# TUMFTM/global_racetrajectory_optimization

Hardware: AMD Instinct MI355X
Metric: min-curv QP solves/sec, N=2000 waypoints, batch=1024 per GPU (higher is better)
Workload: dtype f64

## Files before the change

global_racetrajectory_optimization_amd/csrc/mcq_kernels.hip:

```cpp
#include "mcq_kernels.h"

#include <math.h>



#define MCQ_NT 256
#define MCQ_NW (MCQ_NT / 64)
typedef double d2 __attribute__((vector_size(16)));
typedef __attribute__((address_space(1))) d2 gd2;

#define SM_RED 0
#define SM_S (SM_RED + 64)
#define SPK 1920
#define SM_OVL (SM_S + SPK)
#define OVL_SIZE 7464
#define SM_KV (SM_OVL + OVL_SIZE)
#define SM_KI (SM_KV + 3 * MCQ_KMAX)
#define SM_TOTAL (SM_KI + (3 * MCQ_KMAX + 2 + 1) / 2 + 1)
static_assert(sizeof(double) * SM_TOTAL <= 80 * 1024, "two workgroups of the solver kernel per CU");

size_t mcq_solve_lds_bytes() { return sizeof(double) * SM_TOTAL; }

__shared__ double g_sm[SM_TOTAL];

// ... 425 lines not shown
    if (c.direct) { (void)sp_solve(c, v, v); return; }
    if (c.kkt_f32) solve_kkt<true>(c, v, fwd_done);
    else solve_kkt<false>(c, v, fwd_done);
}

__device__ __forceinline__ void apply_Et(const LCtx& c, const gdouble* src, gdouble* dst) { tri_apply_Et(c, src, dst); }

__device__ __noinline__ void gradient(const LCtx& c, const gdouble* x, const gdouble* extra, gdouble* tmp, gdouble* g)
{
    const int n = c.d.n;
    const long long t0 = TICK();
    __syncthreads();
    if (c.direct) {
        const gdouble* HD = VEC(c.w, c.nm, V_SPD);
        const gdouble* HU = VEC(c.w, c.nm, V_SPU);
        const gdouble* F = VEC(c.w, c.nm, V_F);
        for (int i = threadIdx.x; i < n; i += MCQ_NT) {
            const int im = i > 0 ? i - 1 : n - 1, ip = i + 1 < n ? i + 1 : 0;
            g[i] = F[i] + HU[im] * x[im] + HD[i] * x[i] + HU[i] * x[ip];
        }
        __syncthreads();
        if (threadIdx.x == 0) c.tk[2] += TICK() - t0;
        return;
    }
    tri_apply_E(c, x, VEC(c.w, c.nm, V_KREF), MCQ_F_SCALE, tmp);
    if (extra) {
        for (int i = threadIdx.x; i < n; i += MCQ_NT) tmp[i] += extra[i];
        __syncthreads();
    }
    tri_apply_Et(c, tmp, g);
    if (threadIdx.x == 0) c.tk[2] += TICK() - t0;
}

__device__ __forceinline__ int timed_factor(const LCtx& c, const gdouble* sig, const gschar* mk, gdouble* fv = nullptr, bool f32 = false)
{
    const long long t0 = TICK();
    const int r = factor(c, sig, mk, fv, f32);
    if (threadIdx.x == 0) c.tk[0] += TICK() - t0;
    return r;
}
__device__ __forceinline__ void timed_solve(const LCtx& c, gdouble* v, bool fwd_done = false)
{
    const long long t0 = TICK();
    solve(c, v, fwd_done);
    if (threadIdx.x == 0) c.tk[1] += TICK() - t0;
}


__device__ __noinline__ int ipm(const LCtx& c, bool with_kappa)
{
    const int tid = threadIdx.x, n = c.d.n, nm = c.nm;
    double* red = g_sm + SM_RED;
    const gdouble* LO = VEC(c.w, nm, V_LO);
    const gdouble* HI = VEC(c.w, nm, V_HI);
    const gdouble* KR = VEC(c.w, nm, V_KREF);
    gdouble* X = VEC(c.w, nm, V_X);
    gdouble* G = VEC(c.w, nm, V_G);
    gdouble* ZL = VEC(c.w, nm, V_ZL);
    gdouble* ZU = VEC(c.w, nm, V_ZU);
    gdouble* SIG = VEC(c.w, nm, V_SIG);
    gdouble* RHS = VEC(c.w, nm, V_RHS);
    gdouble* DXA = VEC(c.w, nm, V_DXA);
    gdouble* T0 = VEC(c.w, nm, V_T0);
    gdouble* T1 = VEC(c.w, nm, V_T1);
    gdouble* T2 = VEC(c.w, nm, V_T2);
    gdouble* TL = VEC(c.w, nm, V_TL);
    gdouble* TU = VEC(c.w, nm, V_TU);
    gdouble* YL = VEC(c.w, nm, V_YL);
    gdouble* YU = VEC(c.w, nm, V_YU);
    gdouble* SK = VEC(c.w, nm, V_SK);
    gdouble* EDA = VEC(c.w, nm, V_EDA);
    gdouble* Q = VEC(c.w, nm, V_Q);
    gschar* ST = c.w.state;
    const double kb = c.kbound, zscale = c.zscale;
    const double IPM_TOL = 1e-10;
    c.out_iters = 0;

    for (int i = tid; i < n; i += MCQ_NT) {
        const bool fixed = !(HI[i] - LO[i] > 1e-12);
        ST[i] = fixed ? 2 : 0;
        X[i] = 0.5 * (LO[i] + HI[i]);
        ZL[i] = fixed ? 0.0 : zscale;
        ZU[i] = ZL[i];
    }
    __syncthreads();
    if (with_kappa) {
        tri_apply_E(c, X, KR, 1.0, T0);
        const double mu0 = 0.5 * zscale * c.wmean;
        for (int i = tid; i < n; i += MCQ_NT) {
            const double r = T0[i];
            const double tl = fmax(kb + r, 0.1 * kb), tu = fmax(kb - r, 0.1 * kb);
            TL[i] = tl; TU[i] = tu;
            YL[i] = mu0 / tl; YU[i] = mu0 / tu;
        }
        __syncthreads();
    }
    const double npairs = 2.0 * c.nfree + (with_kappa ? 2.0 * n : 0.0);
    const gschar* const no_mask = nullptr;
    const bool any_fixed = c.nfree < (double)n;
    (void)no_mask;
    if (!(npairs > 0.0)) return MCQ_OK;

    bool g_exact = true;
    double mu_first = 0.0, rdm_best = 1e300;
    for (int it = 1; it <= c.max_ipm_iter; ++it) {
        if (with_kappa) {
            for (int i = tid; i < n; i += MCQ_NT) Q[i] = YU[i] - YL[i];
            gradient(c, X, Q, T0, T1);
            gradient(c, X, nullptr, T0, G);
            tri_apply_E(c, X, KR, 1.0, T0);
        }
        double mu, rdm, rhom;
        for (;;) {
            mu = 0.0; rdm = 0.0; rhom = 0.0;
            for (int i = tid; i < n; i += MCQ_NT) {
                if (with_kappa) {
                    mu += TL[i] * YL[i] + TU[i] * YU[i];
                    rhom = fmax(rhom, fmax(fabs(TL[i] - (kb + T0[i])), fabs(TU[i] - (kb - T0[i]))));
                    SK[i] = YL[i] / TL[i] + YU[i] / TU[i];
                }
                if (ST[i] != 0) continue;
                const double sl = X[i] - LO[i], su = HI[i] - X[i];
                mu += sl * ZL[i] + su * ZU[i];
                const double gg = with_kappa ? T1[i] : G[i];
                rdm = fmax(rdm, fabs(gg - ZL[i] + ZU[i]));
                SIG[i] = ZL[i] / sl + ZU[i] / su;
            }
            mu = block_reduce_(mu, 0, red) / npairs;
            rdm = block_reduce_(rdm, 2, red);
            rhom = block_reduce_(rhom, 2, red);
            const bool conv = mu < IPM_TOL * zscale * c.wmean && rdm < IPM_TOL * zscale && rhom <= 1e-9 * kb;
            if (with_kappa && it > 1 && mu < 1e-6 * mu_first && rdm > 10.0 * rdm_best) return MCQ_OK;
            rdm_best = fmin(rdm_best, rdm);
#ifdef IPM_TRACE
            if (tid == 0) printf("ipm%d it %d mu %.3e rdm %.3e rhom %.3e step %.3e\n", (int)with_kappa, it, mu / (zscale * c.wmean), rdm / zscale, rhom / kb, c.last_step);
#endif
            if (conv && (with_kappa || g_exact)) return MCQ_OK;
            if (!conv) break;
            gradient(c, X, nullptr, T0, G);
            g_exact = true;
        }
        c.out_iters = it;
        if (it == 1) mu_first = mu;

        int fs;
        if (with_kappa) {
            for (int i = tid; i < n; i += MCQ_NT) EDA[i] = 1.0 + SK[i];
            __syncthreads();
            c.kkt_w = EDA;
            fs = timed_factor(c, SIG, any_fixed ? ST : nullptr);
            c.kkt_w = nullptr;
            if (fs == MCQ_NOT_PD && mu < 1e-6 * mu_first) return MCQ_OK;
        } else {
            fs = timed_factor(c, SIG, any_fixed ? ST : nullptr);
        }
        if (fs != 0) return fs;

        if (with_kappa) {
            for (int i = tid; i < n; i += MCQ_NT) {
                const double rl = TL[i] - (kb + T0[i]), ru = TU[i] - (kb - T0[i]);
                Q[i] = YL[i] * rl / TL[i] - YU[i] * ru / TU[i];
            }
            __syncthreads();
            apply_Et(c, Q, T2);
            __syncthreads();
            for (int i = tid; i < n; i += MCQ_NT) RHS[i] = ST[i] == 0 ? -G[i] + T2[i] : 0.0;
        } else {
            for (int i = tid; i < n; i += MCQ_NT) RHS[i] = ST[i] == 0 ? -G[i] : 0.0;
        }
        timed_solve(c, RHS);
        if (with_kappa) {
            tri_apply_E(c, RHS, nullptr, 0.0, EDA);
        }
        double ap = 1.0, ad = 1.0;
        for (int i = tid; i < n; i += MCQ_NT) {
            if (with_kappa) {
                const double rl = TL[i] - (kb + T0[i]), ru = TU[i] - (kb - T0[i]);
                const double dtl = EDA[i] - rl, dtu = -EDA[i] - ru;
                const double dyl = -YL[i] - YL[i] * dtl / TL[i], dyu = -YU[i] - YU[i] * dtu / TU[i];
                if (dtl < 0.0) ap = fmin(ap, -TL[i] / dtl);
                if (dtu < 0.0) ap = fmin(ap, -TU[i] / dtu);
                if (dyl < 0.0) ad = fmin(ad, -YL[i] / dyl);
                if (dyu < 0.0) ad = fmin(ad, -YU[i] / dyu);
            }
            if (ST[i] != 0) { DXA[i] = 0.0; continue; }
            const double dx = RHS[i];
            DXA[i] = dx;
            const double sl = X[i] - LO[i], su = HI[i] - X[i];
            const double dzl = -ZL[i] - ZL[i] * dx / sl, dzu = -ZU[i] + ZU[i] * dx / su;
            if (dx < 0.0) ap = fmin(ap, -sl / dx);
            if (dx > 0.0) ap = fmin(ap, su / dx);
            if (dzl < 0.0) ad = fmin(ad, -ZL[i] / dzl);
            if (dzu < 0.0) ad = fmin(ad, -ZU[i] / dzu);
        }
        ap = block_reduce_(ap, 1, red);
        ad = block_reduce_(ad, 1, red);
        double mua = 0.0;
        for (int i = tid; i < n; i += MCQ_NT) {
            if (with_kappa) {
                const double rl = TL[i] - (kb + T0[i]), ru = TU[i] - (kb - T0[i]);
                const double dtl = EDA[i] - rl, dtu = -EDA[i] - ru;
                const double dyl = -YL[i] - YL[i] * dtl / TL[i], dyu = -YU[i] - YU[i] * dtu / TU[i];
                mua += (TL[i] + ap * dtl) * (YL[i] + ad * dyl) + (TU[i] + ap * dtu) * (YU[i] + ad * dyu);
            }
            if (ST[i] != 0) continue;
            const double dx = DXA[i];
            const double sl = X[i] - LO[i], su = HI[i] - X[i];
            const double dzl = -ZL[i] - ZL[i] * dx / sl, dzu = -ZU[i] + ZU[i] * dx / su;
            mua += (sl + ap * dx) * (ZL[i] + ad * dzl) + (su - ap * dx) * (ZU[i] + ad * dzu);
        }
        mua = block_reduce_(mua, 0, red) / npairs;
        const double ratio = mua / mu;
        const double smu = ratio * ratio * ratio * mu;

        if (with_kappa) {
            for (int i = tid; i < n; i += MCQ_NT) {
                const double rl = TL[i] - (kb + T0[i]), ru = TU[i] - (kb - T0[i]);
                const double dtl = EDA[i] - rl, dtu = -EDA[i] - ru;
                const double dyl = -YL[i] - YL[i] * dtl / TL[i], dyu = -YU[i] - YU[i] * dtu / TU[i];
                Q[i] = (smu - dtl * dyl + YL[i] * rl) / TL[i] - (smu - dtu * dyu + YU[i] * ru) / TU[i];
            }
            __syncthreads();
            apply_Et(c, Q, T2);
            __syncthreads();
        }
        for (int i = tid; i < n; i += MCQ_NT) {
            if (ST[i] != 0) { RHS[i] = 0.0; continue; }
            const double dx = DXA[i];
            const double sl = X[i] - LO[i], su = HI[i] - X[i];
            const double dzl = -ZL[i] - ZL[i] * dx / sl, dzu = -ZU[i] + ZU[i] * dx / su;
            RHS[i] = -G[i] + (smu - dx * dzl) / sl - (smu + dx * dzu) / su + (with_kappa ? T2[i] : 0.0);
        }
        timed_solve(c, RHS);
        if (with_kappa) {
            tri_apply_E(c, RHS, nullptr, 0.0, Q);
        }
        double amax = 1.0 / 0.995;
        for (int i = tid; i < n; i += MCQ_NT) {
            if (with_kappa) {
                const double rl = TL[i] - (kb + T0[i]), ru = TU[i] - (kb - T0[i]);
                const double dtla = EDA[i] - rl, dtua = -EDA[i] - ru;
                const double dyla = -YL[i] - YL[i] * dtla / TL[i], dyua = -YU[i] - YU[i] * dtua / TU[i];
                const double dtl = Q[i] - rl, dtu = -Q[i] - ru;
                const double dyl = (-TL[i] * YL[i] + smu - dtla * dyla - YL[i] * dtl) / TL[i];
                const double dyu = (-TU[i] * YU[i] + smu - dtua * dyua - YU[i] * dtu) / TU[i];
                EDA[i] = dyl;
                SK[i] = dyu;
                if (dtl < 0.0) amax = fmin(amax, -TL[i] / dtl);
                if (dtu < 0.0) amax = fmin(amax, -TU[i] / dtu);
                if (dyl < 0.0) amax = fmin(amax, -YL[i] / dyl);
                if (dyu < 0.0) amax = fmin(amax, -YU[i] / dyu);
            }
            if (ST[i] != 0) continue;
            const double dx = RHS[i], da = DXA[i];
            const double sl = X[i] - LO[i], su = HI[i] - X[i];
            const double dzla = -ZL[i] - ZL[i] * da / sl, dzua = -ZU[i] + ZU[i] * da / su;
            const double dzl = (-sl * ZL[i] + smu - da * dzla - ZL[i] * dx) / sl;
            const double dzu = (-su * ZU[i] + smu + da * dzua + ZU[i] * dx) / su;
            T1[i] = dzl;
            T2[i] = dzu;
            if (dx < 0.0) amax = fmin(amax, -sl / dx);
            if (dx > 0.0) amax = fmin(amax, su / dx);
            if (dzl < 0.0) amax = fmin(amax, -ZL[i] / dzl);
            if (dzu < 0.0) amax = fmin(amax, -ZU[i] / dzu);
        }
        amax = block_reduce_(amax, 1, red);
        const double a = fmin(1.0, 0.995 * amax);
        c.last_step = a;
        for (int i = tid; i < n; i += MCQ_NT) {
            if (with_kappa) {
                const double rl = TL[i] - (kb + T0[i]), ru = TU[i] - (kb - T0[i]);
                TL[i] += a * (Q[i] - rl);
                TU[i] += a * (-Q[i] - ru);
                YL[i] += a * EDA[i];
                YU[i] += a * SK[i];
            }
            if (ST[i] != 0) continue;
            if (!with_kappa) {
                const double dxa = DXA[i], dx = RHS[i];
                const double sl = X[i] - LO[i], su = HI[i] - X[i];
                const double dzla = -ZL[i] - ZL[i] * dxa / sl, dzua = -ZU[i] + ZU[i] * dxa / su;
                const double rc = -G[i] + (smu - dxa * dzla) / sl - (smu + dxa * dzua) / su;
                G[i] += a * (rc - SIG[i] * dx);
            }
            {
                const double sl = X[i] - LO[i], su = HI[i] - X[i];
                const double rsl = (sl + a * RHS[i]) * ZL[i], rzl = (ZL[i] + a * T1[i]) * sl;
                const double rsu = (su - a * RHS[i]) * ZU[i], rzu = (ZU[i] + a * T2[i]) * su;
                const bool al = rsl < MCQ_TAPIA_RATIO * rzl && sl + a * RHS[i] < MCQ_TAPIA_SHRINK * sl, au = rsu < MCQ_TAPIA_RATIO * rzu && su - a * RHS[i] < MCQ_TAPIA_SHRINK * su;
                VEC(c.w, nm, V_T3)[i] = al ? -1.0 : (au ? 1.0 : 0.0);
            }
            X[i] += a * RHS[i];
            ZL[i] += a * T1[i];
            ZU[i] += a * T2[i];
        }
        g_exact = false;
        __syncthreads();
    }
    return with_kappa ? MCQ_KAPPA_INFEASIBLE : MCQ_ITER_CAP;
}

#define IPB_E 8
#define IPB_H 4
__device__ __noinline__ int ipm_box(const LCtx& c, double tol, bool resume)
{
#define IPB_SETUP                                                                                                      \
    const int tid = threadIdx.x, n = c.d.n, nm = c.nm;                                                                 \
    double* red = g_sm + SM_RED;                                                                                       \
    const gdouble* LO = VEC(c.w, nm, V_LO);                                                                            \
    const gdouble* HI = VEC(c.w, nm, V_HI);                                                                            \
    gdouble* X = VEC(c.w, nm, V_X);                                                                                    \
    gdouble* G = VEC(c.w, nm, V_G);                                                                                    \
    gdouble* ZL = VEC(c.w, nm, V_ZL);                                                                                  \
    gdouble* ZU = VEC(c.w, nm, V_ZU);                                                                                  \
    gdouble* SIG = VEC(c.w, nm, V_SIG);                                                                                \
    gdouble* RHS = VEC(c.w, nm, V_RHS);                                                                                \
    gdouble* DXA = VEC(c.w, nm, V_DXA);                                                                                \
    gschar* ST = c.w.state;                                                                                            \
    gdouble* IND = VEC(c.w, nm, V_T3);                                                                                 \
    (void)IND; (void)red; (void)LO; (void)HI; (void)X; (void)G; (void)ZL; (void)ZU; (void)SIG; (void)RHS; (void)DXA; (void)ST;    \
    int idx[IPB_E];                                                                                                    \
    bool ok[IPB_E];                                                                                                    \
    _Pragma("unroll") for (int u = 0; u < IPB_E; ++u) {                                                                \
        ok[u] = tid + u * MCQ_NT < n;                                                                                  \
        idx[u] = ok[u] ? tid + u * MCQ_NT : 0;           \
    }
#define IPB_HALF(h)                                                                                                    \
    int idx[IPB_H];                                                                                                    \
    bool ok[IPB_H];                                                                                                    \
    _Pragma("unroll") for (int u = 0; u < IPB_H; ++u) {                                                                \
        ok[u] = tid + ((h) * IPB_H + u) * MCQ_NT < n;                                                                  \
        idx[u] = ok[u] ? tid + ((h) * IPB_H + u) * MCQ_NT : 0;                                                         \
    }
#define IPB_PTRS                                                                                                       \
    const int tid = threadIdx.x, n = c.d.n, nm = c.nm;                                                                 \
    double* red = g_sm + SM_RED;                                                                                       \
    const gdouble* LO = VEC(c.w, nm, V_LO);                                                                            \
    const gdouble* HI = VEC(c.w, nm, V_HI);                                                                            \
    gdouble* X = VEC(c.w, nm, V_X);                                                                                    \
    gdouble* G = VEC(c.w, nm, V_G);                                                                                    \
    gdouble* ZL = VEC(c.w, nm, V_ZL);                                                                                  \
    gdouble* ZU = VEC(c.w, nm, V_ZU);                                                                                  \
    gdouble* SIG = VEC(c.w, nm, V_SIG);                                                                                \
    gdouble* RHS = VEC(c.w, nm, V_RHS);                                                                                \
    gdouble* DXA = VEC(c.w, nm, V_DXA);                                                                                \
    gschar* ST = c.w.state;                                                                                            \
    gdouble* IND = VEC(c.w, nm, V_T3);                                                                                 \
    (void)IND; (void)red; (void)LO; (void)HI; (void)X; (void)G; (void)ZL; (void)ZU; (void)SIG; (void)RHS; (void)DXA; (void)ST;
    const double zscale = c.zscale;
    const double IPM_TOL = tol;
    c.out_iters = 0;
    {
    IPB_SETUP
#pragma unroll
    for (int u = 0; u < IPB_E; ++u) {
        if (!ok[u]) continue;
        const int i = idx[u];
        const bool fixed = !(HI[i] - LO[i] > 1e-12);
        ST[i] = fixed ? 2 : 0;
        if (!resume) {
            X[i] = 0.5 * (LO[i] + HI[i]);
            ZL[i] = fixed ? 0.0 : zscale;
            ZU[i] = ZL[i];
        }
    }
    }
    __syncthreads();
    if (resume) gradient(c, VEC(c.w, c.nm, V_X), nullptr, VEC(c.w, c.nm, V_T0), VEC(c.w, c.nm, V_G));
    const double npairs = 2.0 * c.nfree;
    const bool any_fixed = c.nfree < (double)c.d.n;
    if (!(npairs > 0.0)) return MCQ_OK;

    bool g_exact = true;
    double mu_prev = 1e300;
    int stalled = 0;
#ifndef MCQ_IPM_F32
#define MCQ_IPM_F32 1
#endif
#ifndef MCQ_IPM_F32_RD
#define MCQ_IPM_F32_RD 1e-5
#endif
    bool f32 = MCQ_IPM_F32 && !resume;
#ifndef MCQ_IPM_TRUST_FP64_CARRY
#define MCQ_IPM_TRUST_FP64_CARRY 1
#endif
    bool g_f32 = false;
    for (int it = 1; it <= c.max_ipm_iter; ++it) {
        double mu;
        for (;;) {
            IPB_PTRS
            double rdm = 0.0;
            mu = 0.0;
            {
#pragma unroll
            for (int h = 0; h < IPB_E / IPB_H; ++h) {
                IPB_HALF(h)
                double x[IPB_H], lo[IPB_H], hi[IPB_H], zl[IPB_H], zu[IPB_H], g[IPB_H];
                int st[IPB_H];
#pragma unroll
                for (int u = 0; u < IPB_H; ++u) {
                    const int i = idx[u];
                    st[u] = ST[i]; x[u] = X[i]; lo[u] = LO[i]; hi[u] = HI[i]; zl[u] = ZL[i]; zu[u] = ZU[i]; g[u] = G[i];
                }
#pragma unroll
                for (int u = 0; u < IPB_H; ++u) {
                    if (!ok[u]) continue;
                    const int i = idx[u];
                    if (st[u] != 0) { RHS[i] = 0.0; continue; }
                    const double sl = x[u] - lo[u], su = hi[u] - x[u];
                    mu += sl * zl[u] + su * zu[u];
                    rdm = fmax(rdm, fabs(g[u] - zl[u] + zu[u]));
                    SIG[i] = zl[u] / sl + zu[u] / su;
                    RHS[i] = -g[u];
                }
            }
            block_reduce2_(mu, 0, rdm, 2, red);
            mu /= npairs;
            }
            const bool conv = mu < IPM_TOL * zscale * c.wmean && rdm < IPM_TOL * zscale;
#ifdef IPM_TRACE
            if (threadIdx.x == 0) printf("ipmb it %d mu %.3e rdm %.3e exact %d resume %d\n", it, mu / (zscale * c.wmean), rdm / zscale, (int)g_exact, (int)resume);
#endif
            if (f32 && it > 1 && rdm < MCQ_IPM_F32_RD * zscale) {
                f32 = false;
                if (!g_exact) {
                    gradient(c, X, nullptr, VEC(c.w, nm, V_T0), G);
                    g_exact = true;
                    g_f32 = false;
                    continue;
                }
            }
            if (conv && (g_exact || (MCQ_IPM_TRUST_FP64_CARRY && !resume && !g_f32))) return MCQ_OK;
            if (!conv) break;
            gradient(c, X, nullptr, VEC(c.w, nm, V_T0), G);
            g_exact = true;
            g_f32 = false;
        }
        c.out_iters = it;
        if (resume) {
            stalled = mu > 0.9 * mu_prev ? stalled + 1 : 0;
            mu_prev = mu;
            if (stalled >= 3) return MCQ_OK;
        }

        const int fs = timed_factor(c, VEC(c.w, c.nm, V_SIG), any_fixed ? c.w.state : nullptr,
                                    VEC(c.w, c.nm, V_RHS), f32);
        if (fs != 0) return (resume && fs == MCQ_NOT_PD) ? MCQ_OK : fs;
        timed_solve(c, VEC(c.w, c.nm, V_RHS), true);

        double smu;
        {
            IPB_SETUP
            double dxa[IPB_E], sl[IPB_E], su[IPB_E], zl[IPB_E], zu[IPB_E], g[IPB_E];
            bool act[IPB_E];
#pragma unroll
            for (int u = 0; u < IPB_E; ++u) {
                const int i = idx[u];
                const double x = X[i];
                act[u] = ok[u] && ST[i] == 0;
                dxa[u] = RHS[i]; sl[u] = x - LO[i]; su[u] = HI[i] - x; zl[u] = ZL[i]; zu[u] = ZU[i]; g[u] = G[i];
            }
            double ap = 1.0, ad = 1.0;
#pragma unroll
            for (int u = 0; u < IPB_E; ++u) {
                if (!ok[u]) continue;
                if (!act[u]) { DXA[idx[u]] = 0.0; continue; }
                const double dx = dxa[u];
                DXA[idx[u]] = dx;
                const double dzla = -zl[u] - zl[u] * dx / sl[u];
                const double dzua = -zu[u] + zu[u] * dx / su[u];
                if (dx < 0.0) ap = fmin(ap, -sl[u] / dx);
                if (dx > 0.0) ap = fmin(ap, su[u] / dx);
                if (dzla < 0.0) ad = fmin(ad, -zl[u] / dzla);
                if (dzua < 0.0) ad = fmin(ad, -zu[u] / dzua);
            }
            block_reduce2_(ap, 1, ad, 1, red);
            double mua = 0.0;
#pragma unroll
            for (int u = 0; u < IPB_E; ++u) {
                if (!act[u]) continue;
                const double dzla = -zl[u] - zl[u] * dxa[u] / sl[u];
                const double dzua = -zu[u] + zu[u] * dxa[u] / su[u];
                mua += (sl[u] + ap * dxa[u]) * (zl[u] + ad * dzla) + (su[u] - ap * dxa[u]) * (zu[u] + ad * dzua);
            }
            mua = block_reduce_(mua, 0, red) / npairs;
            const double ratio = mua / mu;
            smu = ratio * ratio * ratio * mu;
#pragma unroll
            for (int u = 0; u < IPB_E; ++u) {
                if (!ok[u]) continue;
                const double dzla = -zl[u] - zl[u] * dxa[u] / sl[u];
                const double dzua = -zu[u] + zu[u] * dxa[u] / su[u];
                RHS[idx[u]] = act[u] ? -g[u] + (smu - dxa[u] * dzla) / sl[u] - (smu + dxa[u] * dzua) / su[u] : 0.0;
            }
        }
        timed_solve(c, VEC(c.w, c.nm, V_RHS));

        {
            IPB_SETUP
#ifdef MCQ_IPM_FIXED_STEP
            const double gm = 0.995;
#else
            const double gm = fmin(fmax(MCQ_IPM_GM_MIN, 1.0 - MCQ_IPM_GM_C * mu / (zscale * c.wmean)), 1.0 - 1e-9);
#endif
            double amax = 1.0 / gm;
            double dx[IPB_E], da[IPB_E], x[IPB_E], lo[IPB_E], hi[IPB_E], zl[IPB_E], zu[IPB_E], g[IPB_E], sg[IPB_E];
            bool act[IPB_E];
#pragma unroll
            for (int u = 0; u < IPB_E; ++u) {
                const int i = idx[u];
                act[u] = ok[u] && ST[i] == 0;
                dx[u] = RHS[i]; da[u] = DXA[i]; x[u] = X[i]; lo[u] = LO[i]; hi[u] = HI[i]; zl[u] = ZL[i]; zu[u] = ZU[i];
                g[u] = G[i]; sg[u] = SIG[i];
            }
#define IPB_STEP3(u)                                                                                                          \
                const double sl = x[u] - lo[u], su = hi[u] - x[u];                                                              \
                const double dzla = -zl[u] - zl[u] * da[u] / sl, dzua = -zu[u] + zu[u] * da[u] / su;                             \
                const double dzl = (-sl * zl[u] + smu - da[u] * dzla - zl[u] * dx[u]) / sl;                                     \
                const double dzu = (-su * zu[u] + smu + da[u] * dzua + zu[u] * dx[u]) / su;
#pragma unroll
            for (int u = 0; u < IPB_E; ++u) {
                if (!act[u]) continue;
                IPB_STEP3(u)
                if (dx[u] < 0.0) amax = fmin(amax, -sl / dx[u]);
                if (dx[u] > 0.0) amax = fmin(amax, su / dx[u]);
                if (dzl < 0.0) amax = fmin(amax, -zl[u] / dzl);
                if (dzu < 0.0) amax = fmin(amax, -zu[u] / dzu);
            }
            amax = block_reduce_(amax, 1, red);
            const double a = fmin(1.0, gm * amax);
            c.last_step = a;
#pragma unroll
            for (int u = 0; u < IPB_E; ++u) {
                if (!act[u]) continue;
                const int i = idx[u];
                IPB_STEP3(u)
                const double rc = -g[u] + (smu - da[u] * dzla) / sl - (smu + da[u] * dzua) / su;
                const double hdx = rc - sg[u] * dx[u];
                const double gn = g[u] + a * hdx, xn = x[u] + a * dx[u], zln = zl[u] + a * dzl, zun = zu[u] + a * dzu;
                G[i] = gn;
                X[i] = xn;
                ZL[i] = zln;
                ZU[i] = zun;
                const double rsl = (sl + a * dx[u]) * zl[u], rzl = (zl[u] + a * dzl) * sl;
                const double rsu = (su - a * dx[u]) * zu[u], rzu = (zu[u] + a * dzu) * su;
                const bool al = rsl < MCQ_TAPIA_RATIO * rzl && sl + a * dx[u] < MCQ_TAPIA_SHRINK * sl, au = rsu < MCQ_TAPIA_RATIO * rzu && su - a * dx[u] < MCQ_TAPIA_SHRINK * su;
                IND[i] = al ? -1.0 : (au ? 1.0 : 0.0);
            }
#undef IPB_STEP3
        }
        g_exact = false;
        g_f32 |= f32;
        __syncthreads();
    }
    return MCQ_ITER_CAP;
#undef IPB_SETUP
}

struct KappaMem {
    double* kmu;
    double* krh;
    double* mul;
    int* ki;
    int* piv;
    gdouble* sg;
    int cap, ld;
    bool in_lds;
};
__device__ __forceinline__ KappaMem kappa_mem_lds(const LCtx& c)
{
    KappaMem k;
    k.kmu = g_sm + SM_KV;
    k.krh = g_sm + SM_KV + MCQ_KMAX;
    k.mul = g_sm + SM_KV + 2 * MCQ_KMAX;
    k.ki = (int*)(g_sm + SM_KI);
    k.piv = (int*)(g_sm + SM_KI) + 1 + 2 * MCQ_KMAX;
    k.sg = c.w.Z + c.nm;
    k.cap = MCQ_KMAX;
    k.ld = MCQ_KMAX;
    k.in_lds = true;
    return k;
}
__device__ __forceinline__ KappaMem kappa_mem_slot(double* slot)
{
    KappaMem k;
    k.sg = (gdouble*)slot;
    double* v = slot + (size_t)MCQ_KBIG * MCQ_KBIG;
    k.kmu = v;
    k.krh = v + MCQ_KBIG;
    k.mul = v + 2 * MCQ_KBIG;
    k.ki = (int*)(v + 3 * MCQ_KBIG);
    k.piv = k.ki + 2 + 2 * MCQ_KBIG;
    k.cap = MCQ_KBIG;
    k.ld = MCQ_KBIG;
    k.in_lds = false;
    return k;
}

template <typename PA>
__device__ __forceinline__ void kappa_lu_eliminate(PA A, int lda, int nk, double* mul, int* piv)
{
    const int tid = threadIdx.x;
    double* red = g_sm + SM_RED;
    for (int cidx = 0; cidx < nk; ++cidx) {
        double best = -1.0;
        int brow = cidx;
        for (int r = cidx + tid; r < nk; r += MCQ_NT) {
            const double v = fabs(A[(size_t)r * lda + cidx]);
            if (v > best) { best = v; brow = r; }
        }
        const double bmax = block_reduce_(best, 2, red);
        double cand = (best == bmax && best >= 0.0) ? (double)brow : 1e300;
        cand = block_reduce_(cand, 1, red);
        const int pr = cand < 1e299 ? (int)cand : cidx;
        if (tid == 0) piv[cidx] = pr;
        if (pr != cidx)
            for (int cc = tid; cc < nk; cc += MCQ_NT) {
                const double t = A[(size_t)cidx * lda + cc];
                A[(size_t)cidx * lda + cc] = A[(size_t)pr * lda + cc];
                A[(size_t)pr * lda + cc] = t;
            }
        __syncthreads();
        const double pv = A[(size_t)cidx * lda + cidx];
        for (int r = cidx + 1 + tid; r < nk; r += MCQ_NT) mul[r] = pv != 0.0 ? A[(size_t)r * lda + cidx] / pv : 0.0;
        __syncthreads();
        const int rem = nk - cidx - 1;
        for (int e = tid; e < rem * rem; e += MCQ_NT) {
            const int r = cidx + 1 + e / rem, cc = cidx + 1 + e % rem;
            A[(size_t)r * lda + cc] -= mul[r] * A[(size_t)cidx * lda + cc];
        }
        __syncthreads();
        for (int r = cidx + 1 + tid; r < nk; r += MCQ_NT) A[(size_t)r * lda + cidx] = mul[r];
        __syncthreads();
    }
}

__device__ void kappa_lu_factor(const KappaMem& K, int nk)
{
    const int tid = threadIdx.x;
    __syncthreads();
    if (K.in_lds && nk * nk <= OVL_SIZE) {
        double* A = g_sm + SM_OVL;
        for (int e = tid; e < nk * nk; e += MCQ_NT) A[e] = K.sg[(size_t)(e / nk) * K.ld + (e % nk)];
        __syncthreads();
        kappa_lu_eliminate(A, nk, nk, K.mul, K.piv);
        for (int e = tid; e < nk * nk; e += MCQ_NT) K.sg[(size_t)(e / nk) * K.ld + (e % nk)] = A[e];
    } else {
        kappa_lu_eliminate(K.sg, K.ld, nk, K.mul, K.piv);
    }
    __syncthreads();
}

template <typename PA>
__device__ __forceinline__ void kappa_lu_substitute(PA A, int lda, int nk, double* KMU, const int* piv)
{
    const int tid = threadIdx.x;
    if (tid == 0)
        for (int cidx = 0; cidx < nk; ++cidx) {
            const int pr = piv[cidx];
            if (pr != cidx) { const double t = KMU[cidx]; KMU[cidx] = KMU[pr]; KMU[pr] = t; }
        }
    __syncthreads();
    for (int cidx = 0; cidx < nk; ++cidx) {
        const double yc = KMU[cidx];
        __syncthreads();
        for (int r = cidx + 1 + tid; r < nk; r += MCQ_NT) KMU[r] -= A[(size_t)r * lda + cidx] * yc;
        __syncthreads();
    }
    for (int cidx = nk - 1; cidx >= 0; --cidx) {
        if (tid == 0) { const double pv = A[(size_t)cidx * lda + cidx]; KMU[cidx] = pv != 0.0 ? KMU[cidx] / pv : 0.0; }
        __syncthreads();
        const double xc = KMU[cidx];
        for (int r = tid; r < cidx; r += MCQ_NT) KMU[r] -= A[(size_t)r * lda + cidx] * xc;
        __syncthreads();
    }
}

__device__ void kappa_lu_solve(const KappaMem& K, int nk)
{
    const int tid = threadIdx.x;
    __syncthreads();
    for (int q = tid; q < nk; q += MCQ_NT) K.kmu[q] = K.krh[q];
    if (K.in_lds && nk * nk <= OVL_SIZE) {
        double* A = g_sm + SM_OVL;
        for (int e = tid; e < nk * nk; e += MCQ_NT) A[e] = K.sg[(size_t)(e / nk) * K.ld + (e % nk)];
        __syncthreads();
        kappa_lu_substitute((const double*)A, nk, nk, K.kmu, K.piv);
    } else {
        __syncthreads();
        kappa_lu_substitute((const gdouble*)K.sg, K.ld, nk, K.kmu, K.piv);
    }
}

__device__ void kappa_apply(const LCtx& c, const KappaMem& K, int nk, gdouble* Q, gdouble* v)
{
    const int tid = threadIdx.x, n = c.d.n;
    const double* KMU = K.kmu;
    const int* KI = K.ki;
    const gschar* ST = c.w.state;
    for (int i = tid; i < n; i += MCQ_NT) Q[i] = 0.0;
    __syncthreads();
    for (int q = tid; q < nk; q += MCQ_NT) Q[KI[1 + q]] = KMU[q];
    __syncthreads();
    apply_Et(c, Q, v);
    __syncthreads();
    for (int i = tid; i < n; i += MCQ_NT) if (ST[i] != 0) v[i] = 0.0;
    __syncthreads();
    timed_solve(c, v);
}

__device__ __noinline__ int active_set(const LCtx& c, bool with_kappa, bool tapia, int cap, int identify, const KappaMem K)
{
    const int tid = threadIdx.x, n = c.d.n, nm = c.nm;
    double* red = g_sm + SM_RED;
    double* KMU = K.kmu;
    double* KRH = K.krh;
    int* KI = K.ki;
    const int kcap = K.cap;
    const gdouble* LO = VEC(c.w, nm, V_LO);
    const gdouble* HI = VEC(c.w, nm, V_HI);
    const gdouble* KR = VEC(c.w, nm, V_KREF);
    gdouble* X = VEC(c.w, nm, V_X);
    gdouble* G = VEC(c.w, nm, V_G);
    gdouble* ZL = VEC(c.w, nm, V_ZL);
    gdouble* ZU = VEC(c.w, nm, V_ZU);
    gdouble* RHS = VEC(c.w, nm, V_RHS);
    gdouble* T0 = VEC(c.w, nm, V_T0);
    gdouble* T1 = VEC(c.w, nm, V_T1);
    gdouble* T2 = VEC(c.w, nm, V_T2);
    gdouble* T3 = VEC(c.w, nm, V_T3);
    gdouble* Q = VEC(c.w, nm, V_Q);
    gdouble* KF = VEC(c.w, nm, V_SK);
    gdouble* PV = VEC(c.w, nm, V_DXA);
    gschar* ST = c.w.state;
    const double zscale = c.zscale, fscale = c.fscale, kb = c.kbound;
    const int win = MCQ_AS_WINDOW < (n - 1) / 2 ? MCQ_AS_WINDOW : (n - 1) / 2;
    c.out_iters = 0;
    c.out_kkt = 0.0;
    c.out_nk = 0;

    for (int i = tid; i < n; i += MCQ_NT) {
        if (identify == 1 && ST[i] == 0) {
            const double wdt = HI[i] - LO[i];
            const double sl = X[i] - LO[i], su = HI[i] - X[i];
            signed char st = 0;
            if (sl * zscale < ZL[i] * wdt) st = -1;
            else if (su * zscale < ZU[i] * wdt) st = 1;
            if (tapia && st == 0) st = (signed char)VEC(c.w, nm, V_T3)[i];
            ST[i] = st;
        }
        double kf = 0.0;
        if (with_kappa && identify == 2) kf = KF[i];
        else if (with_kappa) {
            const gdouble* TL = VEC(c.w, nm, V_TL);
            const gdouble* TU = VEC(c.w, nm, V_TU);
            const gdouble* YL = VEC(c.w, nm, V_YL);
            const gdouble* YU = VEC(c.w, nm, V_YU);
            const double mu0 = 0.5 * zscale * c.wmean;
            if (TL[i] * mu0 < YL[i] * kb * kb) kf = -1.0;
            else if (TU[i] * mu0 < YU[i] * kb * kb) kf = 1.0;
        }
        KF[i] = kf;
    }
    __syncthreads();
    const double TOLX = 1e-10;
    const double toly = 1e-10 * (fscale > 0.0 ? fscale : 1.0);
    const double tolk = 1e-10 * kb;
    int best = 2 * n + 1, pcnt = 3;
    for (int it = 1; it <= cap; ++it) {
        c.out_iters = it;
        if (tid == 0) {
            int nk = 0;
            if (with_kappa)
                for (int i = 0; i < n; ++i)
                    if (KF[i] != 0.0 && nk < kcap + 1) {
                        if (nk < kcap) { KI[1 + nk] = i; KI[1 + kcap + nk] = KF[i] > 0.0 ? 1 : -1; }
                        ++nk;
                    }
            KI[0] = nk;
        }
        __syncthreads();
        const int nk = KI[0];
        if (nk > kcap) return MCQ_KAPPA_ACTIVE;
        c.out_nk = nk;

        for (int i = tid; i < n; i += MCQ_NT) {
            const signed char st = ST[i];
            T1[i] = st == 0 ? 0.0 : (st < 0 ? LO[i] : (st == 1 ? HI[i] : 0.5 * (LO[i] + HI[i])));
        }
        gradient(c, T1, nullptr, T0, T2);
        for (int i = tid; i < n; i += MCQ_NT) RHS[i] = ST[i] == 0 ? -T2[i] : T1[i];
        const int fs = timed_factor(c, nullptr, ST, RHS);
        if (fs != 0) return fs;
        timed_solve(c, RHS, true);
        if (nk > 0) {
            gdouble* Zs = c.w.Z;
            gdouble* SG = K.sg;
            for (int q = 0; q < nk; ++q) {
                const int k = KI[1 + q];
                for (int i = tid; i < n; i += MCQ_NT) T2[i] = i == k ? 1.0 : 0.0;
                apply_Et(c, T2, Zs);
                for (int i = tid; i < n; i += MCQ_NT) if (ST[i] != 0) Zs[i] = 0.0;
                __syncthreads();
                timed_solve(c, Zs);
                tri_apply_E(c, Zs, nullptr, 0.0, T0);
                for (int q2 = tid; q2 < nk; q2 += MCQ_NT) SG[(size_t)q2 * K.ld + q] = T0[KI[1 + q2]];
                __syncthreads();
            }
            tri_apply_E(c, RHS, KR, 1.0, T0);
            for (int q = tid; q < nk; q += MCQ_NT) KRH[q] = T0[KI[1 + q]] - KI[1 + kcap + q] * kb;
            kappa_lu_factor(K, nk);
            kappa_lu_solve(K, nk);
            kappa_apply(c, K, nk, Q, Zs);
            for (int i = tid; i < n; i += MCQ_NT) RHS[i] -= Zs[i];
            __syncthreads();
        }
        for (int i = tid; i < n; i += MCQ_NT) X[i] = ST[i] == 0 ? RHS[i] : T1[i];
        gradient(c, X, nk > 0 ? Q : nullptr, T0, G);
        if (with_kappa) tri_apply_E(c, X, KR, 1.0, T2);
        double nv = 0.0, imax = -1.0, kk = 0.0;
        for (int i = tid; i < n; i += MCQ_NT) {
            const signed char st = ST[i];
            int v = 0;
            double pv = 0.0;
            if (st == 0) {
                if (X[i] < LO[i] - TOLX) { v = -1; pv = LO[i] - X[i]; }
                else if (X[i] > HI[i] + TOLX) { v = 1; pv = X[i] - HI[i]; }
                kk = fmax(kk, fabs(G[i]));
            } else if (st == -1) { if (G[i] < -toly) v = 2; }
            else if (st == 1) { if (G[i] > toly) v = 2; }
            PV[i] = pv;
            int vk = 0;
            if (with_kappa) {
                const double kf = KF[i];
                if (kf == 0.0) {
                    if (T2[i] > kb + tolk) vk = 1;
                    else if (T2[i] < -kb - tolk) vk = -1;
                } else if (kf * Q[i] < -toly) vk = 2;
            }
            T3[i] = (double)(v + 8 * vk);
            if (v != 0) { nv += 1.0; imax = fmax(imax, (double)i); }
            if (vk != 0) { nv += 1.0; imax = fmax(imax, (double)(n + i)); }
        }
        nv = block_reduce_(nv, 0, red);
        imax = block_reduce_(imax, 2, red);
        c.out_kkt = block_reduce_(kk, 2, red);
        const int nvi = (int)nv;
        if (nvi == 0) {
            for (int r = 0; r < c.refine_steps; ++r) {
                for (int i = tid; i < n; i += MCQ_NT) RHS[i] = ST[i] == 0 ? -G[i] : 0.0;
                timed_solve(c, RHS);
                if (nk > 0) {
                    gdouble* Zs = c.w.Z;
                    tri_apply_E(c, RHS, nullptr, 0.0, T0);
                    for (int q = tid; q < nk; q += MCQ_NT) {
                        const int k = KI[1 + q];
                        KRH[q] = T0[k] + T2[k] - KI[1 + kcap + q] * kb;
                    }
                    kappa_lu_solve(K, nk);
// ... 955 lines not shown
```

Before: 98740.

## Keep box-IPM iterates in registers and defer global writebacks to exit

```diff
diff --git a/global_racetrajectory_optimization_amd/csrc/mcq_kernels.hip b/global_racetrajectory_optimization_amd/csrc/mcq_kernels.hip
--- a/global_racetrajectory_optimization_amd/csrc/mcq_kernels.hip
+++ b/global_racetrajectory_optimization_amd/csrc/mcq_kernels.hip
@@ -751,6 +751,18 @@
 
 #define IPB_E 8
 #define IPB_H 4
+#ifndef MCQ_IPB_RESIDENT
+#define MCQ_IPB_RESIDENT 1
+#endif
+#ifndef MCQ_IPB_DEFER
+#define MCQ_IPB_DEFER MCQ_IPB_RESIDENT
+#endif
+#ifndef MCQ_IPB_NOCOPY
+#define MCQ_IPB_NOCOPY MCQ_IPB_RESIDENT
+#endif
+#if MCQ_IPB_DEFER && !MCQ_IPB_RESIDENT
+#error "MCQ_IPB_DEFER needs MCQ_IPB_RESIDENT"
+#endif
 __device__ __noinline__ int ipm_box(const LCtx& c, double tol, bool resume)
 {
 #define IPB_SETUP                                                                                                      \
@@ -796,6 +808,13 @@
     gschar* ST = c.w.state;                                                                                            \
     gdouble* IND = VEC(c.w, nm, V_T3);                                                                                 \
     (void)IND; (void)red; (void)LO; (void)HI; (void)X; (void)G; (void)ZL; (void)ZU; (void)SIG; (void)RHS; (void)DXA; (void)ST;
+#if MCQ_IPB_NOCOPY
+#define IPB_CORR DXA
+#define IPB_PRED RHS
+#else
+#define IPB_CORR RHS
+#define IPB_PRED DXA
+#endif
     const double zscale = c.zscale;
     const double IPM_TOL = tol;
     c.out_iters = 0;
@@ -819,6 +838,26 @@
     const double npairs = 2.0 * c.nfree;
     const bool any_fixed = c.nfree < (double)c.d.n;
     if (!(npairs > 0.0)) return MCQ_OK;
+#if MCQ_IPB_RESIDENT
+    double rx[IPB_E], rl[IPB_E], ru[IPB_E], rg[IPB_E];
+    {
+        IPB_SETUP
+#pragma unroll
+        for (int u = 0; u < IPB_E; ++u) { const int i = idx[u]; rx[u] = X[i]; rl[u] = ZL[i]; ru[u] = ZU[i]; rg[u] = G[i]; }
+    }
+#define IPB_RELOAD_G { _Pragma("unroll") for (int u = 0; u < IPB_E; ++u) rg[u] = G[tid + u * MCQ_NT < n ? tid + u * MCQ_NT : 0]; }
+#else
+#define IPB_RELOAD_G
+#endif
+#if MCQ_IPB_DEFER
+#define IPB_STORE_X { _Pragma("unroll") for (int u = 0; u < IPB_E; ++u) if (tid + u * MCQ_NT < n) X[tid + u * MCQ_NT] = rx[u]; }
+#define IPB_RETURN(v) { rc = (v); goto ipb_flush; }
+    unsigned tapia = 0;
+    int rc;
+#else
+#define IPB_STORE_X
+#define IPB_RETURN(v) return (v);
+#endif
 
     bool g_exact = true;
     double mu_prev = 1e300;
@@ -849,7 +888,12 @@
 #pragma unroll
                 for (int u = 0; u < IPB_H; ++u) {
                     const int i = idx[u];
+#if MCQ_IPB_RESIDENT
+                    st[u] = ST[i]; lo[u] = LO[i]; hi[u] = HI[i];
+                    x[u] = rx[h * IPB_H + u]; zl[u] = rl[h * IPB_H + u]; zu[u] = ru[h * IPB_H + u]; g[u] = rg[h * IPB_H + u];
+#else
                     st[u] = ST[i]; x[u] = X[i]; lo[u] = LO[i]; hi[u] = HI[i]; zl[u] = ZL[i]; zu[u] = ZU[i]; g[u] = G[i];
+#endif
                 }
 #pragma unroll
                 for (int u = 0; u < IPB_H; ++u) {
@@ -868,20 +912,24 @@
             }
             const bool conv = mu < IPM_TOL * zscale * c.wmean && rdm < IPM_TOL * zscale;
 #ifdef IPM_TRACE
-            if (threadIdx.x == 0) printf("ipmb it %d mu %.3e rdm %.3e exact %d resume %d\n", it, mu / (zscale * c.wmean), rdm / zscale, (int)g_exact, (int)resume);
+            if (threadIdx.x == 0) printf("ipmb it %d mu %.3e rdm %.3e exact %d resume %d [%a %a]\n", it, mu / (zscale * c.wmean), rdm / zscale, (int)g_exact, (int)resume, mu, rdm);
 #endif
             if (f32 && it > 1 && rdm < MCQ_IPM_F32_RD * zscale) {
                 f32 = false;
                 if (!g_exact) {
+                    IPB_STORE_X
                     gradient(c, X, nullptr, VEC(c.w, nm, V_T0), G);
+                    IPB_RELOAD_G
                     g_exact = true;
                     g_f32 = false;
                     continue;
                 }
             }
-            if (conv && (g_exact || (MCQ_IPM_TRUST_FP64_CARRY && !resume && !g_f32))) return MCQ_OK;
+            if (conv && (g_exact || (MCQ_IPM_TRUST_FP64_CARRY && !resume && !g_f32))) IPB_RETURN(MCQ_OK)
             if (!conv) break;
+            IPB_STORE_X
             gradient(c, X, nullptr, VEC(c.w, nm, V_T0), G);
+            IPB_RELOAD_G
             g_exact = true;
             g_f32 = false;
         }
@@ -889,12 +937,12 @@
         if (resume) {
             stalled = mu > 0.9 * mu_prev ? stalled + 1 : 0;
             mu_prev = mu;
-            if (stalled >= 3) return MCQ_OK;
+            if (stalled >= 3) IPB_RETURN(MCQ_OK)
         }
 
         const int fs = timed_factor(c, VEC(c.w, c.nm, V_SIG), any_fixed ? c.w.state : nullptr,
                                     VEC(c.w, c.nm, V_RHS), f32);
-        if (fs != 0) return (resume && fs == MCQ_NOT_PD) ? MCQ_OK : fs;
+        if (fs != 0) IPB_RETURN((resume && fs == MCQ_NOT_PD) ? MCQ_OK : fs)
         timed_solve(c, VEC(c.w, c.nm, V_RHS), true);
 
         double smu;
@@ -905,17 +953,27 @@
 #pragma unroll
             for (int u = 0; u < IPB_E; ++u) {
                 const int i = idx[u];
+                act[u] = ok[u] && ST[i] == 0;
+#if MCQ_IPB_RESIDENT
+                const double x = rx[u];
+                dxa[u] = RHS[i]; sl[u] = x - LO[i]; su[u] = HI[i] - x; zl[u] = rl[u]; zu[u] = ru[u]; g[u] = rg[u];
+#else
                 const double x = X[i];
-                act[u] = ok[u] && ST[i] == 0;
                 dxa[u] = RHS[i]; sl[u] = x - LO[i]; su[u] = HI[i] - x; zl[u] = ZL[i]; zu[u] = ZU[i]; g[u] = G[i];
+#endif
             }
             double ap = 1.0, ad = 1.0;
 #pragma unroll
             for (int u = 0; u < IPB_E; ++u) {
                 if (!ok[u]) continue;
+#if MCQ_IPB_NOCOPY
+                if (!act[u]) continue;
+                const double dx = dxa[u];
+#else
                 if (!act[u]) { DXA[idx[u]] = 0.0; continue; }
                 const double dx = dxa[u];
                 DXA[idx[u]] = dx;
+#endif
                 const double dzla = -zl[u] - zl[u] * dx / sl[u];
                 const double dzua = -zu[u] + zu[u] * dx / su[u];
                 if (dx < 0.0) ap = fmin(ap, -sl[u] / dx);
@@ -940,10 +998,10 @@
                 if (!ok[u]) continue;
                 const double dzla = -zl[u] - zl[u] * dxa[u] / sl[u];
                 const double dzua = -zu[u] + zu[u] * dxa[u] / su[u];
-                RHS[idx[u]] = act[u] ? -g[u] + (smu - dxa[u] * dzla) / sl[u] - (smu + dxa[u] * dzua) / su[u] : 0.0;
-            }
-        }
-        timed_solve(c, VEC(c.w, c.nm, V_RHS));
+                IPB_CORR[idx[u]] = act[u] ? -g[u] + (smu - dxa[u] * dzla) / sl[u] - (smu + dxa[u] * dzua) / su[u] : 0.0;
+            }
+        }
+        timed_solve(c, VEC(c.w, c.nm, MCQ_IPB_NOCOPY ? V_DXA : V_RHS));
 
         {
             IPB_SETUP
@@ -959,8 +1017,12 @@
             for (int u = 0; u < IPB_E; ++u) {
                 const int i = idx[u];
                 act[u] = ok[u] && ST[i] == 0;
-                dx[u] = RHS[i]; da[u] = DXA[i]; x[u] = X[i]; lo[u] = LO[i]; hi[u] = HI[i]; zl[u] = ZL[i]; zu[u] = ZU[i];
-                g[u] = G[i]; sg[u] = SIG[i];
+                dx[u] = IPB_CORR[i]; da[u] = IPB_PRED[i]; lo[u] = LO[i]; hi[u] = HI[i]; sg[u] = SIG[i];
+#if MCQ_IPB_RESIDENT
+                x[u] = rx[u]; zl[u] = rl[u]; zu[u] = ru[u]; g[u] = rg[u];
+#else
+                x[u] = X[i]; zl[u] = ZL[i]; zu[u] = ZU[i]; g[u] = G[i];
+#endif
             }
 #define IPB_STEP3(u)                                                                                                          \
                 const double sl = x[u] - lo[u], su = hi[u] - x[u];                                                              \
@@ -979,6 +1041,11 @@
             amax = block_reduce_(amax, 1, red);
             const double a = fmin(1.0, gm * amax);
             c.last_step = a;
+#if MCQ_IPB_DEFER
+            unsigned t3[IPB_E];
+#pragma unroll
+            for (int u = 0; u < IPB_E; ++u) t3[u] = 0;
+#endif
 #pragma unroll
             for (int u = 0; u < IPB_E; ++u) {
                 if (!act[u]) continue;
@@ -987,23 +1054,61 @@
                 const double rc = -g[u] + (smu - da[u] * dzla) / sl - (smu + da[u] * dzua) / su;
                 const double hdx = rc - sg[u] * dx[u];
                 const double gn = g[u] + a * hdx, xn = x[u] + a * dx[u], zln = zl[u] + a * dzl, zun = zu[u] + a * dzu;
+#if MCQ_IPB_RESIDENT
+                rg[u] = gn; rx[u] = xn; rl[u] = zln; ru[u] = zun;
+#endif
+#if !MCQ_IPB_DEFER
                 G[i] = gn;
                 X[i] = xn;
                 ZL[i] = zln;
                 ZU[i] = zun;
+#endif
                 const double rsl = (sl + a * dx[u]) * zl[u], rzl = (zl[u] + a * dzl) * sl;
                 const double rsu = (su - a * dx[u]) * zu[u], rzu = (zu[u] + a * dzu) * su;
                 const bool al = rsl < MCQ_TAPIA_RATIO * rzl && sl + a * dx[u] < MCQ_TAPIA_SHRINK * sl, au = rsu < MCQ_TAPIA_RATIO * rzu && su - a * dx[u] < MCQ_TAPIA_SHRINK * su;
+#if MCQ_IPB_DEFER
+                t3[u] = al ? 1u : (au ? 3u : 2u);
+                (void)i;
+#else
                 IND[i] = al ? -1.0 : (au ? 1.0 : 0.0);
-            }
+#endif
+            }
+#if MCQ_IPB_DEFER
+            tapia = 0;
+#pragma unroll
+            for (int u = 0; u < IPB_E; ++u) tapia |= t3[u] << (2 * u);
+#endif
 #undef IPB_STEP3
         }
         g_exact = false;
         g_f32 |= f32;
         __syncthreads();
     }
+#if MCQ_IPB_DEFER
+    rc = MCQ_ITER_CAP;
+ipb_flush:
+    {
+        IPB_SETUP
+#pragma unroll
+        for (int u = 0; u < IPB_E; ++u) {
+            if (!ok[u]) continue;
+            const int i = idx[u];
+            X[i] = rx[u]; ZL[i] = rl[u]; ZU[i] = ru[u]; G[i] = rg[u];
+            const unsigned t = (tapia >> (2 * u)) & 3u;
+            if (t != 0) IND[i] = (double)((int)t - 2);
+        }
+    }
+    __syncthreads();
+    return rc;
+#else
     return MCQ_ITER_CAP;
+#endif
 #undef IPB_SETUP
+#undef IPB_RELOAD_G
+#undef IPB_STORE_X
+#undef IPB_RETURN
+#undef IPB_CORR
+#undef IPB_PRED
 }
 
 struct KappaMem {
```

Measured after the change: 102,100, median of 6. 3.4% higher.
